# wenyuqing/panacea

Measured on AMD Instinct MI355X. Metric: denoising steps/s (6-view x 8-frame 256x512), higher is better.
Workload: dtype f16; 1 GPU; BASELINE config 3: Panacea+ stage-2 UNet+ControlNet, CFG 2 x 8 frames, 6 views, latent 32x384, hint 256x3072, Euler/LegacyDDPM 50-step schedule; precision=precise: split(stream,gn_stt,ff_out,stem,gn_head,gnt)+e4m3-lo, parallelism=single, graph=False, streams=2, hoisted_step_invariants=False, fused_step_tail=True

## Files before the change

panacea_amd/csrc/norm.hip:

```cpp
#include "common.h"
#include <type_traits>

namespace {

constexpr int GROUPS = 32;


__device__ __forceinline__ int gn_wave_pixels(int np, int w) { return np > w ? (np - w + 3) >> 2 : 0; }

template <int J>
__device__ __forceinline__ bool gn_reduce_records(float* sm, int Cs, int cpg, int ng, int np, const float2 (&pv)[J],
                                                  const f32x4 (&sum)[J], const f32x4 (&sq)[J], float& n, float& mean, float& m2) {
    const int tid = threadIdx.x, lane = tid & 63, wave = tid >> 6;
    const int CVs = Cs >> 2;
    float* mine = sm + wave * Cs;
    float* s_gmean = sm + 4 * Cs;
    const float nw = (float)gn_wave_pixels(np, wave);
    const float inw = nw > 0.0f ? 1.0f / nw : 0.0f;
    const float icpg = 1.0f / (float)cpg;
    f32x4 m[J];
#pragma unroll
    for (int j = 0; j < J; ++j) {
        const int cv = lane + j * 64;
#pragma unroll
        for (int e = 0; e < 4; ++e) m[j][e] = fmaf(sum[j][e], inw, e < 2 ? pv[j].x : pv[j].y);
        if (cv < CVs) *reinterpret_cast<f32x4*>(mine + cv * 4) = m[j];
    }
    __syncthreads();
    n = (float)np * (float)cpg;
    mean = 0.0f; m2 = 0.0f;
    if (tid < ng) {
        const float P = sm[tid * cpg];
        float acc = 0.0f;
        for (int w = 0; w < 4; ++w) {
            const float k = (float)gn_wave_pixels(np, w);
            float a = 0.0f;
            for (int c = 0; c < cpg; ++c) a += sm[w * Cs + tid * cpg + c] - P;
            acc = fmaf(k, a, acc);
        }
        mean = P + acc / n;
        s_gmean[tid] = mean;
    }
    __syncthreads();
#pragma unroll
    for (int j = 0; j < J; ++j) {
        const int cv = lane + j * 64;
        if (cv < CVs) {
            f32x4 r;
#pragma unroll
            for (int e = 0; e < 4; ++e) {
                const float dm = m[j][e] - s_gmean[(int)(((float)(cv * 4 + e) + 0.5f) * icpg)];
                r[e] = fmaf(nw * dm, dm, fmaxf(fmaf(-sum[j][e] * inw, sum[j][e], sq[j][e]), 0.0f));
            }
            *reinterpret_cast<f32x4*>(mine + cv * 4) = r;
        }
    }
    __syncthreads();
    if (tid < ng)
        for (int w = 0; w < 4; ++w)
            for (int c = 0; c < cpg; ++c) m2 += sm[w * Cs + tid * cpg + c];
    return tid < ng;
}

template <int J>
__global__ __launch_bounds__(256) void gn_stats_kernel(const float* __restrict__ x, int ldx, int Npix, int C,
                                                       int ppc, float* __restrict__ partial) {
    extern __shared__ __attribute__((aligned(16))) float sm[];
    const int f = blockIdx.y, chunk = blockIdx.x, nchunk = gridDim.x;
    const int tid = threadIdx.x, lane = tid & 63, wave = tid >> 6;
    const int CV = C >> 2, cpg = C / GROUPS;
    const int p0 = chunk * ppc;
    const int p1 = min(Npix, p0 + ppc);
    f32x4 sum[J], sq[J];
    float2 pv[J];
    const f32x4 z = {0.0f, 0.0f, 0.0f, 0.0f};
#pragma unroll
    for (int j = 0; j < J; ++j) { sum[j] = z; sq[j] = z; pv[j] = make_float2(0.0f, 0.0f); }
    if (p0 + wave < p1) {
        const float* row = x + ((int64_t)f * Npix + p0 + wave) * ldx;
#pragma unroll
        for (int j = 0; j < J; ++j) {
            const int cv = lane + j * 64;
            if (cv < CV) {
                const f32x4 v = *reinterpret_cast<const f32x4*>(row + cv * 4);
                pv[j] = make_float2(v[0], v[2]);
                sum[j] = f32x4{0.0f, v[1] - v[0], 0.0f, v[3] - v[2]};
                sq[j] = sum[j] * sum[j];
            }
        }
    }
#pragma unroll 2
    for (int pix = p0 + wave + 4; pix < p1; pix += 4) {
        const float* row = x + ((int64_t)f * Npix + pix) * ldx;
        f32x4 v[J];
#pragma unroll
        for (int j = 0; j < J; ++j) {
            const int cv = lane + j * 64;
            v[j] = (cv < CV) ? *reinterpret_cast<const f32x4*>(row + cv * 4) : z;
        }
#pragma unroll
        for (int j = 0; j < J; ++j) {
            const f32x4 d = v[j] - f32x4{pv[j].x, pv[j].x, pv[j].y, pv[j].y};
            sum[j] += d;
#pragma unroll
            for (int e = 0; e < 4; ++e) sq[j][e] = fmaf(d[e], d[e], sq[j][e]);
        }
    }
    float n, mean, m2;
    if (gn_reduce_records<J>(sm, C, cpg, GROUPS, p1 - p0, pv, sum, sq, n, mean, m2)) {
        float* o = partial + ((int64_t)(f * nchunk + chunk) * GROUPS + tid) * 3;
        o[0] = n; o[1] = mean; o[2] = m2;
    }
}

template <int J>
__global__ __launch_bounds__(256) void gn_apply_kernel(const float* __restrict__ x, int ldx, int Npix, int C,
                                                       int ppc, const float* __restrict__ partial,
                                                       const float* __restrict__ gamma,
                                                       const float* __restrict__ beta, float eps, int silu,
                                                       half_t* __restrict__ y, int ldy, void* __restrict__ ylo, int lo_fmt, int nrec) {
    extern __shared__ __attribute__((aligned(16))) float sm[];
    const int tabw = 2 * C > 24 * GROUPS ? 2 * C : 24 * GROUPS;
    float* sA = sm;
    float* sB = sm + C;
    float* s_mean = sm + tabw;
    float* s_rstd = s_mean + GROUPS;
    const int f = blockIdx.y, chunk = blockIdx.x, nchunk = nrec;
    const int tid = threadIdx.x, lane = tid & 63, wave = tid >> 6;
    {
        float* s_pn = sm;
        float* s_pm = sm + 8 * GROUPS;
        float* s_p2 = sm + 16 * GROUPS;
        const int g = tid & 31, part = tid >> 5;
        float n = 0.0f, mean = 0.0f, m2 = 0.0f;
        for (int c = part; c < nchunk; c += 8) {
            const float* q = partial + ((int64_t)(f * nchunk + c) * GROUPS + g) * 3;
            const float nb = q[0], mb = q[1], m2b = q[2];
            const float nt = n + nb, d = mb - mean;
            const float w = nb / fmaxf(nt, 1.0f);
            mean = fmaf(d, w, mean);
            m2 += m2b + d * d * (n * w);
            n = nt;
        }
        s_pn[part * GROUPS + g] = n; s_pm[part * GROUPS + g] = mean; s_p2[part * GROUPS + g] = m2;
        __syncthreads();
        float fm = 0.0f, fr = 0.0f;
        if (tid < GROUPS) {
            float tn = 0.0f, tm = 0.0f, t2 = 0.0f;
            for (int k = 0; k < 8; ++k) {
                const float nb = s_pn[k * GROUPS + tid], mb = s_pm[k * GROUPS + tid], m2b = s_p2[k * GROUPS + tid];
                const float nt = tn + nb, d = mb - tm;
                const float w = nb / fmaxf(nt, 1.0f);
                tm = fmaf(d, w, tm);
                t2 += m2b + d * d * (tn * w);
                tn = nt;
            }
            fm = tm; fr = rsqrtf(t2 / tn + eps);
        }
        __syncthreads();
        if (tid < GROUPS) { s_mean[tid] = fm; s_rstd[tid] = fr; }
    }
    __syncthreads();
    const int CV = C >> 2, cpg = C / GROUPS;
    for (int c = tid; c < C; c += 256) {
        const int g = c / cpg;
        const float a = gamma[c] * s_rstd[g];
        sA[c] = a;
        sB[c] = fmaf(-s_mean[g], a, beta[c]);
    }
    __syncthreads();
    const int p0 = chunk * ppc;
    const int p1 = min(Npix, p0 + ppc);
    const f32x4 z = {0.0f, 0.0f, 0.0f, 0.0f};
    constexpr int R = J <= 3 ? 4 : (J <= 6 ? 2 : 1);
    for (int pix0 = p0 + wave; pix0 < p1; pix0 += 4 * R) {
        f32x4 v[R][J];
#pragma unroll
        for (int rr = 0; rr < R; ++rr) {
            const int pix = pix0 + 4 * rr;
            const float* row = x + ((int64_t)f * Npix + pix) * ldx;
#pragma unroll
            for (int j = 0; j < J; ++j) {
                const int cv = lane + j * 64;
                v[rr][j] = (cv < CV && pix < p1) ? *reinterpret_cast<const f32x4*>(row + cv * 4) : z;
            }
        }
#pragma unroll
        for (int rr = 0; rr < R; ++rr) {
            const int pix = pix0 + 4 * rr;
            if (pix >= p1) break;
            half_t* yrow = y + ((int64_t)f * Npix + pix) * ldy;
#pragma unroll
            for (int j = 0; j < J; ++j) {
                const int cv = lane + j * 64;
                if (cv < CV) {
                    const f32x4 a = *reinterpret_cast<const f32x4*>(sA + cv * 4);
                    const f32x4 b = *reinterpret_cast<const f32x4*>(sB + cv * 4);
                    half4v h;
                    float o[4];
#pragma unroll
                    for (int e = 0; e < 4; ++e) {
                        o[e] = fmaf(v[rr][j][e], a[e], b[e]);
                        if (silu) o[e] = silu_f(o[e]);
                        h[e] = (half_t)o[e];
                    }
                    *reinterpret_cast<half4v*>(yrow + cv * 4) = h;
                    if (ylo) store_lo4(ylo, lo_fmt, ((int64_t)f * Npix + pix) * ldy + cv * 4, o, h);
                }
            }
        }
    }
}

template <int T, int MODE = 0, int NIT = (T <= 8 ? 2 : 1)>
__global__ __launch_bounds__(512 / NIT) void gn_temporal_kernel(const float* __restrict__ x, int B, int Npix, int C,
                                                          const float* __restrict__ gamma,
                                                          const float* __restrict__ beta, float eps,
                                                          half_t* __restrict__ y, void* __restrict__ ylo, int lo_fmt, int PB,
                                                          float* __restrict__ stats = nullptr, int T_total = T, int t_pad = 0) {
    extern __shared__ __attribute__((aligned(16))) float sm[];
    const int CP = C >> 1, C4 = C >> 2, cpg2 = (C / GROUPS) >> 1;
    float* s_part = sm;
    float* s_stat = sm + (size_t)PB * CP * 2;
    const int tid = threadIdx.x;
    const int64_t bp0 = (int64_t)blockIdx.x * PB;
    const int64_t total = (int64_t)B * Npix;
    const int nwork = PB * C4;
    constexpr int NT = 512 / NIT;
    f32x4 v[NIT][T];
    int64_t off[NIT], offo[NIT];
    bool live[NIT];
#pragma unroll
    for (int it = 0; it < NIT; ++it) {
        const int wi = tid + it * NT;
        const int pl = wi / C4, c4 = wi - pl * C4;
        const int64_t bp = bp0 + pl;
        live[it] = (wi < nwork) && (bp < total);
        float s0 = 0.0f, q0 = 0.0f, s1 = 0.0f, q1 = 0.0f;
        off[it] = 0; offo[it] = 0;
        if (live[it]) {
            const int64_t b = bp / Npix, pix = bp - b * Npix;
            off[it] = ((b * T) * Npix + pix) * C + c4 * 4;
            offo[it] = ((b * (T + 2 * t_pad) + t_pad) * Npix + pix) * C + c4 * 4;
#pragma unroll
            for (int t = 0; t < T; ++t) v[it][t] = *reinterpret_cast<const f32x4*>(x + off[it] + (int64_t)t * Npix * C);
            if constexpr (MODE == 0) {
                const float pa = v[it][0][0], pb = v[it][0][2];
#pragma unroll
                for (int t = 0; t < T; ++t) {
                    s0 += (v[it][t][0] - pa) + (v[it][t][1] - pa);
                    s1 += (v[it][t][2] - pb) + (v[it][t][3] - pb);
                }
                s0 = fmaf(s0, 1.0f / (float)(2 * T), pa);
                s1 = fmaf(s1, 1.0f / (float)(2 * T), pb);
            } else {
#pragma unroll
                for (int t = 0; t < T; ++t) {
                    s0 += v[it][t][0] + v[it][t][1]; q0 = fmaf(v[it][t][0], v[it][t][0], q0); q0 = fmaf(v[it][t][1], v[it][t][1], q0);
                    s1 += v[it][t][2] + v[it][t][3]; q1 = fmaf(v[it][t][2], v[it][t][2], q1); q1 = fmaf(v[it][t][3], v[it][t][3], q1);
                }
            }
        }
        if (wi < nwork) {
            float* d = s_part + ((size_t)pl * CP + c4 * 2) * 2;
            d[0] = s0; d[2] = s1;
            if constexpr (MODE != 0) { d[1] = q0; d[3] = q1; }
        }
    }
    __syncthreads();
    if constexpr (MODE == 0) {
        for (int gi = tid; gi < PB * GROUPS; gi += NT) {
            const int pl = gi / GROUPS, g = gi - pl * GROUPS;
            const float P = s_part[(pl * CP + g * cpg2) * 2];
            float s = 0.0f;
            for (int j = 0; j < cpg2; ++j) s += s_part[(pl * CP + g * cpg2 + j) * 2] - P;
            s_stat[gi * 2] = P + s / (float)cpg2;
        }
        __syncthreads();
#pragma unroll
        for (int it = 0; it < NIT; ++it) {
            const int wi = tid + it * NT;
            if (wi >= nwork) continue;
            const int pl = wi / C4, c4 = wi - pl * C4;
            float q0 = 0.0f, q1 = 0.0f;
            if (live[it]) {
                const float ma = s_stat[(pl * GROUPS + (c4 * 2) / cpg2) * 2], mb = s_stat[(pl * GROUPS + (c4 * 2 + 1) / cpg2) * 2];
#pragma unroll
                for (int t = 0; t < T; ++t) {
                    const float d0 = v[it][t][0] - ma, d1 = v[it][t][1] - ma, d2 = v[it][t][2] - mb, d3 = v[it][t][3] - mb;
                    q0 = fmaf(d0, d0, q0); q0 = fmaf(d1, d1, q0);
                    q1 = fmaf(d2, d2, q1); q1 = fmaf(d3, d3, q1);
                }
            }
            float* d = s_part + ((size_t)pl * CP + c4 * 2) * 2;
            d[1] = q0; d[3] = q1;
        }
        __syncthreads();
        for (int gi = tid; gi < PB * GROUPS; gi += NT) {
            const int pl = gi / GROUPS, g = gi - pl * GROUPS;
            float q = 0.0f;
            for (int j = 0; j < cpg2; ++j) q += s_part[(pl * CP + g * cpg2 + j) * 2 + 1];
            s_stat[gi * 2 + 1] = rsqrtf(q / (float)(cpg2 * 2 * T) + eps);
        }
    } else {
        for (int gi = tid; gi < PB * GROUPS; gi += NT) {
            const int pl = gi / GROUPS, g = gi - pl * GROUPS;
            float s = 0.0f, q = 0.0f;
            for (int j = 0; j < cpg2; ++j) {
                const int wi = pl * CP + g * cpg2 + j;
                s += s_part[wi * 2]; q += s_part[wi * 2 + 1];
            }
            if constexpr (MODE == 1) {
                const int64_t bp = bp0 + pl;
                if (bp < total) { stats[(bp * GROUPS + g) * 2] = s; stats[(bp * GROUPS + g) * 2 + 1] = q; }
                continue;
            }
            if constexpr (MODE == 2) {
                const int64_t bp = bp0 + pl;
                if (bp < total) { s = stats[(bp * GROUPS + g) * 2]; q = stats[(bp * GROUPS + g) * 2 + 1]; }
            }
            const float n = (float)(cpg2 * 2 * T_total);
            const float mean = s / n;
            const float var = fmaxf(q / n - mean * mean, 0.0f);
            s_stat[gi * 2] = mean; s_stat[gi * 2 + 1] = rsqrtf(var + eps);
        }
    }
    if constexpr (MODE == 1) return;
    __syncthreads();
#pragma unroll
    for (int it = 0; it < NIT; ++it) {
        if (!live[it]) continue;
        const int wi = tid + it * NT;
        const int pl = wi / C4, c4 = wi - pl * C4;
        const int ga = (c4 * 2) / cpg2, gb = (c4 * 2 + 1) / cpg2;
        const float ma = s_stat[(pl * GROUPS + ga) * 2], ra = s_stat[(pl * GROUPS + ga) * 2 + 1];
        const float mb = s_stat[(pl * GROUPS + gb) * 2], rb = s_stat[(pl * GROUPS + gb) * 2 + 1];
        const f32x4 gm = *reinterpret_cast<const f32x4*>(gamma + c4 * 4);
        const f32x4 bt = *reinterpret_cast<const f32x4*>(beta + c4 * 4);
        const float g0 = gm[0] * ra, g1 = gm[1] * ra, g2 = gm[2] * rb, g3 = gm[3] * rb;
#pragma unroll
        for (int t = 0; t < T; ++t) {
            const float o[4] = {silu_f(fmaf(v[it][t][0] - ma, g0, bt[0])), silu_f(fmaf(v[it][t][1] - ma, g1, bt[1])),
                                silu_f(fmaf(v[it][t][2] - mb, g2, bt[2])), silu_f(fmaf(v[it][t][3] - mb, g3, bt[3]))};
            const half4v h = {(half_t)o[0], (half_t)o[1], (half_t)o[2], (half_t)o[3]};
            *reinterpret_cast<half4v*>(y + offo[it] + (int64_t)t * Npix * C) = h;
            if (ylo) store_lo4(ylo, lo_fmt, offo[it] + (int64_t)t * Npix * C, o, h);
        }
    }
}

constexpr int LN_R = 4;
template <int J>
__global__ __launch_bounds__(256) void layernorm_kernel(const float* __restrict__ x, int ldx, int M, int C,
                                                        const float* __restrict__ gamma,
                                                        const float* __restrict__ beta, float eps,
                                                        half_t* __restrict__ y, int ldy, half_t* __restrict__ ylo) {
    const int lane = threadIdx.x & 63;
    const int64_t row0 = ((int64_t)blockIdx.x * 4 + (threadIdx.x >> 6)) * LN_R;
    if (row0 >= M) return;
    const int CV = C >> 2;
    f32x4 v[LN_R][J];
    const f32x4 z = {0.0f, 0.0f, 0.0f, 0.0f};
#pragma unroll
    for (int r = 0; r < LN_R; ++r) {
        const int64_t row = (row0 + r < M) ? row0 + r : (int64_t)M - 1;
        const float* xr = x + row * ldx;
#pragma unroll
        for (int j = 0; j < J; ++j) {
            const int cv = lane + j * 64;
            v[r][j] = (cv < CV) ? *reinterpret_cast<const f32x4*>(xr + cv * 4) : z;
        }
    }
    f32x4 g[J], b[J];
#pragma unroll
    for (int j = 0; j < J; ++j) {
        const int cv = lane + j * 64;
        g[j] = (cv < CV) ? *reinterpret_cast<const f32x4*>(gamma + cv * 4) : z;
        b[j] = (cv < CV) ? *reinterpret_cast<const f32x4*>(beta + cv * 4) : z;
    }
    float mean[LN_R], rstd[LN_R], corr[LN_R];
    const float invc = 1.0f / (float)C;
#pragma unroll
    for (int r = 0; r < LN_R; ++r) {
        float s = 0.0f;
#pragma unroll
        for (int j = 0; j < J; ++j) s += (v[r][j][0] + v[r][j][1]) + (v[r][j][2] + v[r][j][3]);
        mean[r] = s;
    }
#pragma unroll
    for (int o = 32; o > 0; o >>= 1)
#pragma unroll
        for (int r = 0; r < LN_R; ++r) mean[r] += __shfl_xor(mean[r], o, 64);
#pragma unroll
    for (int r = 0; r < LN_R; ++r) {
        mean[r] *= invc;
        float q = 0.0f, s1 = 0.0f;
#pragma unroll
        for (int j = 0; j < J; ++j) {
            const int cv = lane + j * 64;
            if (cv < CV) {
#pragma unroll
                for (int e = 0; e < 4; ++e) { const float d = v[r][j][e] - mean[r]; q = fmaf(d, d, q); s1 += d; }
            }
        }
        rstd[r] = q; corr[r] = s1;
    }
#pragma unroll
    for (int o = 32; o > 0; o >>= 1)
#pragma unroll
        for (int r = 0; r < LN_R; ++r) { rstd[r] += __shfl_xor(rstd[r], o, 64); corr[r] += __shfl_xor(corr[r], o, 64); }
#pragma unroll
    for (int r = 0; r < LN_R; ++r) {
        const float dm = corr[r] * invc;
        mean[r] += dm;
        rstd[r] = fmaf(-dm, dm, rstd[r] * invc);
    }
#pragma unroll
    for (int r = 0; r < LN_R; ++r) {
        if (row0 + r >= M) break;
        const float rs = rsqrtf(rstd[r] + eps);
        half_t* yr = y + (row0 + r) * ldy;
#pragma unroll
        for (int j = 0; j < J; ++j) {
            const int cv = lane + j * 64;
            if (cv < CV) {
                half4v h;
                float o[4];
#pragma unroll
                for (int e = 0; e < 4; ++e) { o[e] = fmaf((v[r][j][e] - mean[r]) * rs, g[j][e], b[j][e]); h[e] = (half_t)o[e]; }
                *reinterpret_cast<half4v*>(yr + cv * 4) = h;
                if (ylo) *reinterpret_cast<half4v*>(ylo + (row0 + r) * ldy + cv * 4) = lo_plane4(o, h);
            }
        }
    }
}

__global__ __launch_bounds__(256) void gn_combine_kernel(const float* __restrict__ in, int parts, int F, int nchunk,
                                                         float* __restrict__ out) {
    __shared__ float s_pn[8 * GROUPS], s_pm[8 * GROUPS], s_p2[8 * GROUPS];
    const int f = blockIdx.x, tid = threadIdx.x;
    const int g = tid & 31, part = tid >> 5;
    const int nrec = parts * nchunk;
    float n = 0.0f, mean = 0.0f, m2 = 0.0f;
    for (int r = part; r < nrec; r += 8) {
        const int s = r / nchunk, c = r - s * nchunk;
        const float* q = in + ((((int64_t)s * F + f) * nchunk + c) * GROUPS + g) * 3;
        const float nb = q[0], mb = q[1], m2b = q[2];
        const float nt = n + nb, d = mb - mean;
        const float w = nb / fmaxf(nt, 1.0f);
        mean = fmaf(d, w, mean);
        m2 += m2b + d * d * (n * w);
        n = nt;
    }
    s_pn[part * GROUPS + g] = n; s_pm[part * GROUPS + g] = mean; s_p2[part * GROUPS + g] = m2;
    __syncthreads();
    if (tid < GROUPS) {
        float tn = 0.0f, tm = 0.0f, t2 = 0.0f;
        for (int k = 0; k < 8; ++k) {
            const float nb = s_pn[k * GROUPS + tid], mb = s_pm[k * GROUPS + tid], m2b = s_p2[k * GROUPS + tid];
            const float nt = tn + nb, d = mb - tm;
            const float w = nb / fmaxf(nt, 1.0f);
            tm = fmaf(d, w, tm);
            t2 += m2b + d * d * (tn * w);
            tn = nt;
        }
        float* o = out + ((int64_t)f * nchunk * GROUPS + tid) * 3;
        o[0] = tn; o[1] = tm; o[2] = t2;
    }
    for (int i = GROUPS * 3 + tid; i < nchunk * GROUPS * 3; i += 256) out[(int64_t)f * nchunk * GROUPS * 3 + i] = 0.0f;
}

template <int J>
__global__ __launch_bounds__(256) void concat_add_stats_kernel(const float* __restrict__ a, int C1, const float* __restrict__ s,
                                                               const float* __restrict__ c, int C2, int Npix, int ppc,
                                                               float* __restrict__ out32, half_t* __restrict__ out16,
                                                               void* __restrict__ out16_lo, int lo_fmt, float* __restrict__ partial) {
    extern __shared__ __attribute__((aligned(16))) float sm[];
    const int f = blockIdx.y, chunk = blockIdx.x, nchunk = gridDim.x, S = gridDim.z, z = blockIdx.z;
    const int tid = threadIdx.x, lane = tid & 63, wave = tid >> 6;
    const int C = C1 + C2, cpg = C / GROUPS;
    const int Cs = C / S, c0 = z * Cs, CVs = Cs >> 2, gps = GROUPS / S;
    const int p0 = chunk * ppc;
    const int p1 = min(Npix, p0 + ppc);
    f32x4 sum[J], sq[J];
    float2 pv[J];
    const f32x4 zz = {0.0f, 0.0f, 0.0f, 0.0f};
#pragma unroll
    for (int j = 0; j < J; ++j) { sum[j] = zz; sq[j] = zz; pv[j] = make_float2(0.0f, 0.0f); }
#pragma unroll 2
    for (int pix = p0 + wave; pix < p1; pix += 4) {
        const int64_t m = (int64_t)f * Npix + pix;
        f32x4 v[J];
#pragma unroll
        for (int j = 0; j < J; ++j) {
            const int cv = lane + j * 64, ch = c0 + cv * 4;
            v[j] = zz;
            if (cv < CVs) {
                if (ch < C1) {
                    v[j] = *reinterpret_cast<const f32x4*>(a + m * C1 + ch);
                } else {
                    v[j] = *reinterpret_cast<const f32x4*>(s + m * C2 + (ch - C1));
                    if (c) v[j] += *reinterpret_cast<const f32x4*>(c + m * C2 + (ch - C1));
                }
            }
        }
        const bool first = pix == p0 + wave;
#pragma unroll
        for (int j = 0; j < J; ++j) {
            const int cv = lane + j * 64, ch = c0 + cv * 4;
            if (cv < CVs) {
                if (out32) *reinterpret_cast<f32x4*>(out32 + m * C + ch) = v[j];
                if (out16) {
                    half4v h = {(half_t)v[j][0], (half_t)v[j][1], (half_t)v[j][2], (half_t)v[j][3]};
                    *reinterpret_cast<half4v*>(out16 + m * C + ch) = h;
                    if (out16_lo) {
                        const float o[4] = {v[j][0], v[j][1], v[j][2], v[j][3]};
                        store_lo4(out16_lo, lo_fmt, m * C + ch, o, h);
                    }
                }
            }
            if (first) pv[j] = make_float2(v[j][0], v[j][2]);
            const f32x4 d = v[j] - f32x4{pv[j].x, pv[j].x, pv[j].y, pv[j].y};
            sum[j] += d;
#pragma unroll
            for (int e = 0; e < 4; ++e) sq[j][e] = fmaf(d[e], d[e], sq[j][e]);
        }
    }
    float n, mean, m2;
    if (gn_reduce_records<J>(sm, Cs, cpg, gps, p1 - p0, pv, sum, sq, n, mean, m2)) {
        float* o = partial + ((int64_t)(f * nchunk + chunk) * GROUPS + z * gps + tid) * 3;
        o[0] = n; o[1] = mean; o[2] = m2;
    }
}

constexpr int GN_MAXC = 4 * 64 * 12;

template <int N> using int_c = std::integral_constant<int, N>;
template <int CAP = 12, typename Launch>
void dispatch_j(int J, Launch&& launch) {
    if (J <= 1) launch(int_c<1>{});
    else if (J == 2) launch(int_c<2>{});
    else if (J == 3 || CAP == 3) launch(int_c<3>{});
    else if constexpr (CAP > 3) {
        if (J <= 5) launch(int_c<5>{});
        else if (J <= 8) launch(int_c<8>{});
        else launch(int_c<12>{});
    }
}
int vectors_per_lane(int C) { return (C / 4 + 63) / 64; }

struct GnTemporalGeom { int PB; unsigned blocks; size_t lds; };
GnTemporalGeom gn_temporal_geom(int B, int Npix, int C) {
    int PB = 512 / (C / 4); if (PB < 1) PB = 1; if (PB > 16) PB = 16;
    return {PB, (unsigned)(((int64_t)B * Npix + PB - 1) / PB), ((size_t)PB * (C / 2) * 2 + (size_t)PB * GROUPS * 2) * sizeof(float)};
}

template <int MODE>
int launch_gn_temporal(int T, void* stream, const float* x, int B, int Npix, int C, const float* gamma, const float* beta, float eps,
                       void* y16, void* y16_lo, int lo_fmt, float* stats, int T_total, int t_pad) {
    if (((uintptr_t)x | (uintptr_t)gamma | (uintptr_t)beta) & 15) return PNC_EALIGN;
    if (((uintptr_t)y16 | (uintptr_t)y16_lo | (uintptr_t)stats) & 7) return PNC_EALIGN;
    const GnTemporalGeom g = gn_temporal_geom(B, Npix, C);
    auto launch = [&](auto frames) {
        constexpr int TT = decltype(frames)::value;
        hipLaunchKernelGGL((gn_temporal_kernel<TT, MODE>), dim3(g.blocks), dim3(TT <= 8 ? 256 : 512), g.lds, reinterpret_cast<hipStream_t>(stream),
                           x, B, Npix, C, gamma, beta, eps, f16p(y16), y16_lo, lo_fmt, g.PB, stats, T_total, t_pad);
    };
    switch (T) {
        case 1: launch(int_c<1>{}); break; case 2: launch(int_c<2>{}); break; case 3: launch(int_c<3>{}); break; case 4: launch(int_c<4>{}); break;
        case 5: launch(int_c<5>{}); break; case 6: launch(int_c<6>{}); break; case 7: launch(int_c<7>{}); break; case 8: launch(int_c<8>{}); break;
        case 9: launch(int_c<9>{}); break; case 10: launch(int_c<10>{}); break; case 11: launch(int_c<11>{}); break; case 12: launch(int_c<12>{}); break;
        case 13: launch(int_c<13>{}); break; case 14: launch(int_c<14>{}); break; case 15: launch(int_c<15>{}); break; case 16: launch(int_c<16>{}); break;
    }
    return pnc_launch_status();
}

}

extern "C" int pnc_groupnorm_stats(const float* x, int ldx, int F, int Npix, int C,
                                   int pix_per_chunk, float* partial, void* stream) {
    if (!x || !partial || F < 1 || Npix < 1 || pix_per_chunk < 1) return PNC_EINVAL;
    if (C % 64 || C > GN_MAXC || ldx % 4) return PNC_EINVAL;
    if ((uintptr_t)x & 15) return PNC_EALIGN;
    const int nchunk = (Npix + pix_per_chunk - 1) / pix_per_chunk;
    const size_t lds = ((size_t)4 * C + GROUPS) * sizeof(float);
    hipStream_t st = reinterpret_cast<hipStream_t>(stream);
    dispatch_j(vectors_per_lane(C), [&](auto j) {
        hipLaunchKernelGGL(gn_stats_kernel<decltype(j)::value>, dim3(nchunk, F), dim3(256), lds, st, x, ldx, Npix, C, pix_per_chunk, partial);
    });
    return pnc_launch_status();
}

extern "C" int pnc_concat_add_stats(const float* a, int C1, const float* s, const float* c, int C2, int F, int Npix, int pix_per_chunk,
                                    float* out32, void* out16, void* out16_lo, int lo_fmt, float* partial, void* stream) {
    if (!a || !s || !partial || F < 1 || Npix < 1 || pix_per_chunk < 1 || C1 % 4 || C2 % 4 || C1 < 4 || C2 < 4) return PNC_EINVAL;
    if (lo_fmt != PNC_LO_F16 && lo_fmt != PNC_LO_E4M3) return PNC_EINVAL;
    if ((!out32 && !out16) || (out16_lo && !out16)) return PNC_EINVAL;
    const int C = C1 + C2;
    if (C % 64 || C > GN_MAXC) return PNC_EINVAL;
    if (((uintptr_t)a | (uintptr_t)s | (uintptr_t)c | (uintptr_t)out32) & 15) return PNC_EALIGN;
    const int nchunk = (Npix + pix_per_chunk - 1) / pix_per_chunk;
    int S = 1;
    while (S < 8 && vectors_per_lane(C / S) > 3 && (C / (2 * S)) % 4 == 0) S *= 2;
    if (vectors_per_lane(C / S) > 3) return PNC_EINVAL;
    const size_t lds = ((size_t)4 * (C / S) + GROUPS) * sizeof(float);
    hipStream_t st = reinterpret_cast<hipStream_t>(stream);
    dispatch_j<3>(vectors_per_lane(C / S), [&](auto j) {
        hipLaunchKernelGGL(concat_add_stats_kernel<decltype(j)::value>, dim3(nchunk, F, S), dim3(256), lds, st, a, C1, s, c, C2, Npix, pix_per_chunk,
                           out32, f16p(out16), out16_lo, lo_fmt, partial);
    });
    return pnc_launch_status();
}

extern "C" int pnc_groupnorm_apply(const float* x, int ldx, int F, int Npix, int C,
                                   int pix_per_chunk, const float* partial,
                                   const float* gamma, const float* beta, float eps, int silu,
                                   void* y16, int ldy, void* y16_lo, int lo_fmt, int n_records, void* stream) {
    if (!x || !partial || !gamma || !beta || !y16 || F < 1 || Npix < 1 || pix_per_chunk < 1 || n_records < 0) return PNC_EINVAL;
    if (lo_fmt != PNC_LO_F16 && lo_fmt != PNC_LO_E4M3) return PNC_EINVAL;
    if (C % 64 || C > GN_MAXC || ldx % 4 || ldy % 4) return PNC_EINVAL;
    if (((uintptr_t)x & 15) || (((uintptr_t)y16 | (uintptr_t)y16_lo) & 7)) return PNC_EALIGN;
    const int nchunk = (Npix + pix_per_chunk - 1) / pix_per_chunk;
    const size_t lds = ((size_t)(2 * C > 24 * GROUPS ? 2 * C : 24 * GROUPS) + 2 * GROUPS) * sizeof(float);
    hipStream_t st = reinterpret_cast<hipStream_t>(stream);
    dispatch_j(vectors_per_lane(C), [&](auto j) {
        hipLaunchKernelGGL(gn_apply_kernel<decltype(j)::value>, dim3(nchunk, F), dim3(256), lds, st, x, ldx, Npix, C, pix_per_chunk, partial,
                           gamma, beta, eps, silu, f16p(y16), ldy, y16_lo, lo_fmt, n_records > 0 ? n_records : nchunk);
    });
    return pnc_launch_status();
}

extern "C" int pnc_groupnorm_combine(const float* in, int parts, int F, int nchunk, float* out, void* stream) {
    if (!in || !out || parts < 1 || F < 1 || nchunk < 1) return PNC_EINVAL;
    hipLaunchKernelGGL(gn_combine_kernel, dim3(F), dim3(256), 0, reinterpret_cast<hipStream_t>(stream), in, parts, F, nchunk, out);
    return pnc_launch_status();
}

extern "C" int pnc_groupnorm_temporal_silu(const float* x, int B, int T, int Npix, int C,
                                           const float* gamma, const float* beta, float eps,
                                           void* y16, void* y16_lo, int lo_fmt, void* stream) {
    if (!x || !gamma || !beta || !y16 || B < 1 || Npix < 1) return PNC_EINVAL;
    if (lo_fmt != PNC_LO_F16 && lo_fmt != PNC_LO_E4M3) return PNC_EINVAL;
    if (C % 64 || C > 2048 || T < 1 || T > 16) return PNC_EINVAL;
    return launch_gn_temporal<0>(T, stream, x, B, Npix, C, gamma, beta, eps, y16, y16_lo, lo_fmt, nullptr, T, 0);
}

extern "C" int pnc_groupnorm_temporal_part(const float* x, int B, int T, int Npix, int C,
                                           const float* gamma, const float* beta, float eps,
                                           float* stats, int mode, int T_total,
                                           void* y16, void* y16_lo, int lo_fmt, int t_pad, void* stream) {
    if (!x || !stats || B < 1 || Npix < 1 || (mode != 1 && mode != 2)) return PNC_EINVAL;
    if (C % 64 || C > 2048 || T < 1 || T > 16 || T_total < T || (t_pad != 0 && t_pad != 1)) return PNC_EINVAL;
    if (mode == 2 && (!gamma || !beta || !y16 || (lo_fmt != PNC_LO_F16 && lo_fmt != PNC_LO_E4M3))) return PNC_EINVAL;
    return (mode == 1 ? launch_gn_temporal<1> : launch_gn_temporal<2>)(T, stream, x, B, Npix, C, gamma, beta, eps, y16, y16_lo, lo_fmt, stats, T_total, t_pad);
}

extern "C" int pnc_layernorm(const float* x, int ldx, int M, int C,
                             const float* gamma, const float* beta, float eps,
                             void* y16, int ldy, void* y16_lo, void* stream) {
    if (!x || !gamma || !beta || !y16 || M < 1) return PNC_EINVAL;
    if (C % 4 || C > 4 * 64 * 12 || C < 4 || ldx % 4 || ldy % 4) return PNC_EINVAL;
    if (((uintptr_t)x | (uintptr_t)gamma | (uintptr_t)beta) & 15) return PNC_EALIGN;
    if (((uintptr_t)y16 | (uintptr_t)y16_lo) & 7) return PNC_EALIGN;
    const unsigned blocks = (unsigned)(((int64_t)M + 4 * LN_R - 1) / (4 * LN_R));
    hipStream_t st = reinterpret_cast<hipStream_t>(stream);
    dispatch_j(vectors_per_lane(C), [&](auto j) {
        hipLaunchKernelGGL(layernorm_kernel<decltype(j)::value>, dim3(blocks), dim3(256), 0, st, x, ldx, M, C, gamma, beta, eps,
                           f16p(y16), ldy, f16p(y16_lo));
    });
    return pnc_launch_status();
}

PNC_DEFINE_TU_COLLECT(norm)
```

Measured before the change: 6.282 steps/s.

## Prefetch first GroupNorm rows before stats merge and specialize lo-store format

The GroupNorm apply kernel now issues the first batch of activation loads before the partial-stat reduction, so global-memory latency overlaps the combine and table setup. The partial-record merge loop is unrolled by four to raise memory-level parallelism. The low-precision side output format becomes a template parameter, removing runtime branches, and the store loop is reordered to reuse the scale/bias loads across rows. The early prefetch keeps more values live in registers through the reduction, which may lower occupancy, and it can be turned off with an option bit.

New measurement: 6.298 steps/s (median of 6 runs). About the same (+0.2%).

```diff
diff --git a/panacea_amd/csrc/norm.hip b/panacea_amd/csrc/norm.hip
--- a/panacea_amd/csrc/norm.hip
+++ b/panacea_amd/csrc/norm.hip
@@ -113,12 +113,15 @@
     }
 }
 
-template <int J>
+template <int J, int LO>
 __global__ __launch_bounds__(256) void gn_apply_kernel(const float* __restrict__ x, int ldx, int Npix, int C,
                                                        int ppc, const float* __restrict__ partial,
                                                        const float* __restrict__ gamma,
                                                        const float* __restrict__ beta, float eps, int silu,
-                                                       half_t* __restrict__ y, int ldy, void* __restrict__ ylo, int lo_fmt, int nrec) {
+                                                       half_t* __restrict__ y, int ldy, void* __restrict__ ylo_arg, int nrec,
+                                                       int early) {
+    void* const ylo = LO ? ylo_arg : nullptr;
+    constexpr int lo_fmt = LO == 2 ? PNC_LO_E4M3 : PNC_LO_F16;
     extern __shared__ __attribute__((aligned(16))) float sm[];
     const int tabw = 2 * C > 24 * GROUPS ? 2 * C : 24 * GROUPS;
     float* sA = sm;
@@ -126,21 +129,57 @@
     float* s_mean = sm + tabw;
     float* s_rstd = s_mean + GROUPS;
     const int f = blockIdx.y, chunk = blockIdx.x, nchunk = nrec;
-    const int tid = threadIdx.x, lane = tid & 63, wave = tid >> 6;
+    const int tid = threadIdx.x, lane = tid & 63, wave = __builtin_amdgcn_readfirstlane(tid >> 6);
+    const unsigned lane4 = lane * 4;
+    const int CV = C >> 2, cpg = C / GROUPS;
+    const int p0 = chunk * ppc;
+    const int p1 = min(Npix, p0 + ppc);
+    const f32x4 z = {0.0f, 0.0f, 0.0f, 0.0f};
+    constexpr int R = J <= 3 ? 4 : (J <= 6 ? 2 : 1);
+    f32x4 v[R][J];
+    auto load_rows = [&](int pix0) {
+#pragma unroll
+        for (int rr = 0; rr < R; ++rr) {
+            const int pix = pix0 + 4 * rr;
+            const float* row = x + ((int64_t)f * Npix + pix) * ldx;
+#pragma unroll
+            for (int j = 0; j < J; ++j) {
+                const int cv = lane + j * 64;
+                v[rr][j] = (cv < CV && pix < p1) ? *reinterpret_cast<const f32x4*>(row + j * 256 + lane4) : z;
+            }
+        }
+    };
+    if (early) load_rows(p0 + wave);
     {
         float* s_pn = sm;
         float* s_pm = sm + 8 * GROUPS;
         float* s_p2 = sm + 16 * GROUPS;
         const int g = tid & 31, part = tid >> 5;
         float n = 0.0f, mean = 0.0f, m2 = 0.0f;
-        for (int c = part; c < nchunk; c += 8) {
-            const float* q = partial + ((int64_t)(f * nchunk + c) * GROUPS + g) * 3;
-            const float nb = q[0], mb = q[1], m2b = q[2];
+        auto merge = [&](float nb, float mb, float m2b) {
             const float nt = n + nb, d = mb - mean;
             const float w = nb / fmaxf(nt, 1.0f);
             mean = fmaf(d, w, mean);
             m2 += m2b + d * d * (n * w);
             n = nt;
+        };
+        if (early) {
+            for (int c = part; c < nchunk; c += 32) {
+                float nb[4], mb[4], m2b[4];
+#pragma unroll
+                for (int u = 0; u < 4; ++u) {
+                    const float* q = partial + ((int64_t)(f * nchunk + min(c + 8 * u, nchunk - 1)) * GROUPS + g) * 3;
+                    nb[u] = q[0]; mb[u] = q[1]; m2b[u] = q[2];
+                }
+#pragma unroll
+                for (int u = 0; u < 4; ++u)
+                    if (c + 8 * u < nchunk) merge(nb[u], mb[u], m2b[u]);
+            }
+        } else {
+            for (int c = part; c < nchunk; c += 8) {
+                const float* q = partial + ((int64_t)(f * nchunk + c) * GROUPS + g) * 3;
+                merge(q[0], q[1], q[2]);
+            }
         }
         s_pn[part * GROUPS + g] = n; s_pm[part * GROUPS + g] = mean; s_p2[part * GROUPS + g] = m2;
         __syncthreads();
@@ -161,7 +200,6 @@
         if (tid < GROUPS) { s_mean[tid] = fm; s_rstd[tid] = fr; }
     }
     __syncthreads();
-    const int CV = C >> 2, cpg = C / GROUPS;
     for (int c = tid; c < C; c += 256) {
         const int g = c / cpg;
         const float a = gamma[c] * s_rstd[g];
@@ -169,33 +207,20 @@
         sB[c] = fmaf(-s_mean[g], a, beta[c]);
     }
     __syncthreads();
-    const int p0 = chunk * ppc;
-    const int p1 = min(Npix, p0 + ppc);
-    const f32x4 z = {0.0f, 0.0f, 0.0f, 0.0f};
-    constexpr int R = J <= 3 ? 4 : (J <= 6 ? 2 : 1);
     for (int pix0 = p0 + wave; pix0 < p1; pix0 += 4 * R) {
-        f32x4 v[R][J];
-#pragma unroll
-        for (int rr = 0; rr < R; ++rr) {
-            const int pix = pix0 + 4 * rr;
-            const float* row = x + ((int64_t)f * Npix + pix) * ldx;
-#pragma unroll
-            for (int j = 0; j < J; ++j) {
-                const int cv = lane + j * 64;
-                v[rr][j] = (cv < CV && pix < p1) ? *reinterpret_cast<const f32x4*>(row + cv * 4) : z;
-            }
-        }
-#pragma unroll
-        for (int rr = 0; rr < R; ++rr) {
-            const int pix = pix0 + 4 * rr;
-            if (pix >= p1) break;
-            half_t* yrow = y + ((int64_t)f * Npix + pix) * ldy;
-#pragma unroll
-            for (int j = 0; j < J; ++j) {
-                const int cv = lane + j * 64;
-                if (cv < CV) {
-                    const f32x4 a = *reinterpret_cast<const f32x4*>(sA + cv * 4);
-                    const f32x4 b = *reinterpret_cast<const f32x4*>(sB + cv * 4);
+        if (!early || pix0 != p0 + wave) load_rows(pix0);
+        constexpr int lo_bytes = lo_fmt == PNC_LO_E4M3 ? 1 : 2;
+        auto y_at = [&](int rr, int j) { return y + ((int64_t)f * Npix + pix0 + 4 * rr) * ldy + j * 256; };
+        auto lo_at = [&](int rr, int j) { return reinterpret_cast<char*>(ylo) + (((int64_t)f * Npix + pix0 + 4 * rr) * ldy + j * 256) * lo_bytes; };
+#pragma unroll
+        for (int j = 0; j < J; ++j) {
+            const int cv = lane + j * 64;
+            if (cv < CV) {
+                const f32x4 a = *reinterpret_cast<const f32x4*>(sA + cv * 4);
+                const f32x4 b = *reinterpret_cast<const f32x4*>(sB + cv * 4);
+#pragma unroll
+                for (int rr = 0; rr < R; ++rr) {
+                    if (pix0 + 4 * rr >= p1) break;
                     half4v h;
                     float o[4];
 #pragma unroll
@@ -204,8 +229,8 @@
                         if (silu) o[e] = silu_f(o[e]);
                         h[e] = (half_t)o[e];
                     }
-                    *reinterpret_cast<half4v*>(yrow + cv * 4) = h;
-                    if (ylo) store_lo4(ylo, lo_fmt, ((int64_t)f * Npix + pix) * ldy + cv * 4, o, h);
+                    *reinterpret_cast<half4v*>(y_at(rr, j) + lane4) = h;
+                    if constexpr (LO != 0) store_lo4(lo_at(rr, j), lo_fmt, lane4, o, h);
                 }
             }
         }
@@ -624,8 +649,14 @@
     const size_t lds = ((size_t)(2 * C > 24 * GROUPS ? 2 * C : 24 * GROUPS) + 2 * GROUPS) * sizeof(float);
     hipStream_t st = reinterpret_cast<hipStream_t>(stream);
     dispatch_j(vectors_per_lane(C), [&](auto j) {
-        hipLaunchKernelGGL(gn_apply_kernel<decltype(j)::value>, dim3(nchunk, F), dim3(256), lds, st, x, ldx, Npix, C, pix_per_chunk, partial,
-                           gamma, beta, eps, silu, f16p(y16), ldy, y16_lo, lo_fmt, n_records > 0 ? n_records : nchunk);
+        const int early = (pnc_get_option(PNC_OPT_GEMM_FUSE_LN) & 512) == 0;
+        auto launch = [&](auto lo) {
+            hipLaunchKernelGGL((gn_apply_kernel<decltype(j)::value, decltype(lo)::value>), dim3(nchunk, F), dim3(256), lds, st, x, ldx, Npix, C,
+                               pix_per_chunk, partial, gamma, beta, eps, silu, f16p(y16), ldy, y16_lo, n_records > 0 ? n_records : nchunk, early);
+        };
+        if (!y16_lo) launch(int_c<0>{});
+        else if (lo_fmt == PNC_LO_F16) launch(int_c<1>{});
+        else launch(int_c<2>{});
     });
     return pnc_launch_status();
 }
```
